# benjiebob/SMALify

Hardware: AMD Instinct MI355X
Metric: fitter iterations/sec (higher is better)
Workload: dtype f32

## Files before the change

### smalify_amd/csrc/kernels_raster.inc

```

#ifdef SMALFIT_DEV_PROBES
#define SMALFIT_PROBE(flags, bit) (((flags) & (bit)) != 0)
#else
#define SMALFIT_PROBE(flags, bit) false
#endif

#ifdef SMALFIT_WORK_STATS
__device__ unsigned long long g_work[32];
__device__ float g_probe_seed_scale;
#define SMALFIT_WORK(...) __VA_ARGS__
__device__ __forceinline__ void work_add(int slot, unsigned long long v) {
  unsigned lo = (unsigned)v, hi = (unsigned)(v >> 32);
#pragma unroll
  for (int o = 32; o > 0; o >>= 1) {
    const unsigned long long w = ((unsigned long long)__shfl_xor(hi, o, 64) << 32) | __shfl_xor(lo, o, 64);
    const unsigned long long s = (((unsigned long long)hi << 32) | lo) + w;
    lo = (unsigned)s; hi = (unsigned)(s >> 32);
  }
  if ((threadIdx.x & 63) == 0) atomicAdd(&g_work[slot], ((unsigned long long)hi << 32) | lo);
}
__device__ __forceinline__ int wave_max_i(int v) {
#pragma unroll
  for (int o = 32; o > 0; o >>= 1) v = max(v, __shfl_xor(v, o, 64));
  return v;
}
#else
#define SMALFIT_WORK(...)
#endif

constexpr int kListCap = 128;
constexpr int kListLds = 128;
static_assert(kListLds <= kListCap && kListLds % 8 == 0, "lists are copied out in 8-byte pieces");
constexpr int kMaskRounds = 64;
constexpr unsigned char kMaskList = 254;
constexpr unsigned char kNoList = 255;
constexpr float kBoxSlack = 1.0f / 64.0f;
constexpr int kTicketBase = 64, kTicketStride = 16;
constexpr int kQCountInts = kTicketBase + 8 * kSelGroups * kTicketStride;
constexpr int kAccWin = 36;
constexpr int kCountShift = 50;
constexpr float kLogFix = 16777216.0f;
constexpr int kBandCap = 64;
constexpr int kBandFill = 24;
constexpr int kBandFillWide = 40, kBandFillNarrow = 12;
constexpr int kBandStage = 64;
constexpr float kBandHalf = 4.0f;

struct SilTarget {
  const float* f;
  const unsigned char* b;
  __host__ __device__ explicit operator bool() const { return f != nullptr || b != nullptr; }
  __device__ __forceinline__ float operator[](size_t i) const { return b ? (float)b[i] / 255.0f : f[i]; }
};

__device__ __forceinline__ void xcd_block_of(int b , int blocks_per_frame, int& n, int& bx) {
  const int xcd = b & 7, slot = b >> 3;
  n = (slot / blocks_per_frame) * 8 + xcd;
  bx = slot - (slot / blocks_per_frame) * blocks_per_frame;
}
__device__ __forceinline__ void xcd_block(int blocks_per_frame, int& n, int& bx) { xcd_block_of((int)blockIdx.x, blocks_per_frame, n, bx); }

__device__ __forceinline__ unsigned orderable(float f) {
  const unsigned u = __float_as_uint(f);
  return (u & 0x80000000u) ? ~u : (u | 0x80000000u);
}
__device__ __forceinline__ float from_orderable(unsigned k) {
  return __uint_as_float((k & 0x80000000u) ? (k & 0x7fffffffu) : ~k);
}
__device__ __forceinline__ float wave_prod(float v) {
#pragma unroll
  for (int o = 32; o > 0; o >>= 1) v *= __shfl_xor(v, o, 64);
  return v;
}
__device__ __forceinline__ bool box_contains(int2 b, int x, int y) {
  return (b.x & 0xffff) <= x && x <= (b.x >> 16) && (b.y & 0xffff) <= y && y <= (b.y >> 16);
}
__device__ __forceinline__ unsigned long long pack_candidate(float d) {
  const float x2 = d * (1.4426950408889634f / kSigma);
  const float t = __builtin_amdgcn_exp2f(-fabsf(x2));
  const float f = fminf(__builtin_amdgcn_logf(1.0f + t) - fminf(x2, 0.0f), 255.99998f);
  return (1ull << kCountShift) | (unsigned long long)(unsigned)fmaf(f, kLogFix, 0.5f);
}

struct PixelSeed { float sil, adiff, gx; };
__device__ __forceinline__ PixelSeed pixel_no_target(float alpha) { return {1.0f - alpha, 0.f, 0.f}; }
__device__ __forceinline__ PixelSeed pixel_seed(float alpha, float ts, float wn) {
  PixelSeed p = pixel_no_target(alpha);
  const float diff = p.sil - ts;
  p.adiff = fabsf(diff);
  const float sgn = (diff > 0.f) ? 1.0f : ((diff < 0.f) ? -1.0f : 0.0f);
  p.gx = -wn * sgn * alpha * (1.0f / kSigma);
  return p;
}

__device__ __forceinline__ float prob_fast(float d) {
  return __builtin_amdgcn_rcpf(1.0f + __builtin_amdgcn_exp2f(d * (1.4426950408889634f / kSigma)));
}

constexpr int kRecVecs = 4;
__device__ __forceinline__ void store_face_rec(float4* __restrict__ o, const FaceRec& r) {
  o[0] = make_float4(r.ax, r.ay, r.e1x, r.e1y);
  o[1] = make_float4(r.e2x, r.e2y, r.e3x, r.e3y);
  o[2] = make_float4(r.il1, r.il2, r.il3, r.area);
  o[3] = make_float4(r.inv_den, r.pz0, r.gzx, r.gzy);
}
__device__ __forceinline__ void unpack_face_rec(const float4 a, const float4 b, const float4 c, const float4 d, FaceRec& r) {
  r.ax = a.x; r.ay = a.y; r.e1x = a.z; r.e1y = a.w;
  r.e2x = b.x; r.e2y = b.y; r.e3x = b.z; r.e3y = b.w;
  r.il1 = c.x; r.il2 = c.y; r.il3 = c.z; r.area = c.w;
  r.t01 = (c.x == 0.0f) ? 1.0f : 0.0f; r.t02 = (c.y == 0.0f) ? 1.0f : 0.0f; r.t03 = (c.z == 0.0f) ? 1.0f : 0.0f;
  r.inv_den = d.x; r.pz0 = d.y; r.gzx = d.z; r.gzy = d.w; r.pad = 0.0f;
}
__device__ __forceinline__ void load_face_rec(const float4* __restrict__ fr, FaceRec& r) {
  const float4 a = fr[0], b = fr[1], c = fr[2], d = fr[3];
  unpack_face_rec(a, b, c, d, r);
}

__global__ void __launch_bounds__(256)
face_bbox_kernel(ModelDev m, int M, int S, const float* __restrict__ proj, int2* __restrict__ fbox,
                 float4* __restrict__ frec , int4* __restrict__ brect ,
                 float* __restrict__ zc , int* __restrict__ frect ,
                 int* __restrict__ qcount ,
                 const float* __restrict__ jverts, float* __restrict__ joints_out ) {
  const int nfr = box_frame_blocks(M);
  const int Vp = m.Vp;
  if ((int)blockIdx.x < nfr) {
    const int n = (int)blockIdx.x;
    if (n >= M) return;
    if (n == 0) {
      if (threadIdx.x < 3) qcount[threadIdx.x] = 0;
      for (int i = threadIdx.x; i < 8 * kSelGroups; i += 256) qcount[kTicketBase + i * kTicketStride] = 0;
    }
    const float* px = proj + (size_t)n * 3 * Vp;
    if (threadIdx.x < 64) {
      const float zsum = wave_sum(px[2 * Vp + (int)(((long long)threadIdx.x * m.V) >> 6)]);
      if (threadIdx.x == 0) zc[n] = zsum * (1.0f / 64.0f);
    }
    __shared__ float rr[4][4];
    float xlo = 3.0e38f, xhi = -3.0e38f, ylo = 3.0e38f, yhi = -3.0e38f;
#pragma unroll 8
    for (int v = threadIdx.x; v < m.V; v += 256) {
      const float x = px[v], y = px[Vp + v];
      xlo = fminf(xlo, x); xhi = fmaxf(xhi, x); ylo = fminf(ylo, y); yhi = fmaxf(yhi, y);
    }
#pragma unroll
    for (int o = 32; o > 0; o >>= 1) {
      xlo = fminf(xlo, __shfl_xor(xlo, o, 64)); xhi = fmaxf(xhi, __shfl_xor(xhi, o, 64));
      ylo = fminf(ylo, __shfl_xor(ylo, o, 64)); yhi = fmaxf(yhi, __shfl_xor(yhi, o, 64));
    }
    if ((threadIdx.x & 63) == 0) { float* q = rr[threadIdx.x >> 6]; q[0] = xlo; q[1] = xhi; q[2] = ylo; q[3] = yhi; }
    __syncthreads();
    if (threadIdx.x == 0) {
      for (int w = 1; w < 4; ++w) { xlo = fminf(xlo, rr[w][0]); xhi = fmaxf(xhi, rr[w][1]); ylo = fminf(ylo, rr[w][2]); yhi = fmaxf(yhi, rr[w][3]); }
      xlo -= kBlurSqrt; xhi += kBlurSqrt; ylo -= kBlurSqrt; yhi += kBlurSqrt;
      const float fs = (float)S;
      const float c0 = fmaxf(floorf(((1.0f - xhi) * fs - 1.0f) * 0.5f), 0.f), c1 = fminf(ceilf(((1.0f - xlo) * fs - 1.0f) * 0.5f), fs - 1.f);
      const float r0 = fmaxf(floorf(((1.0f - yhi) * fs - 1.0f) * 0.5f), 0.f), r1 = fminf(ceilf(((1.0f - ylo) * fs - 1.0f) * 0.5f), fs - 1.f);
      int4 o = make_int4(0, 0, 0, 0);
      if (c0 <= c1 && r0 <= r1) o = make_int4(S - (int)c0, (int)c1 + 1, S - (int)r0, (int)r1 + 1);
      *reinterpret_cast<int4*>(frect + n * 4) = o;
    }
    return;
  }
  const int nbb = box_face_blocks(m.F, M);
  if ((int)blockIdx.x >= nfr + nbb) {
    __shared__ float jred[16];
    const int k = (int)blockIdx.x - nfr - nbb;
    joints_block(m, jverts, joints_out, k % kJointBlocks, k / kJointBlocks, jred);
    return;
  }
  int n, bxi;
  xcd_block_of((int)blockIdx.x - nfr, box_blocks_per_frame(m.F), n, bxi);
  if (n >= M) return;
  __shared__ __attribute__((aligned(16))) float4 recs[256][kRecVecs];
  const int f = bxi * 256 + threadIdx.x;
  const float* px = proj + (size_t)n * 3 * Vp;
  int2 box = make_int2(1, 1);
  if (f < m.F) {
    const int i0 = m.faces[f * 3], i1 = m.faces[f * 3 + 1], i2 = m.faces[f * 3 + 2];
    const float ax = px[i0], ay = px[Vp + i0], az = px[2 * Vp + i0];
    const float bx = px[i1], by = px[Vp + i1], bz = px[2 * Vp + i1];
    const float cx = px[i2], cy = px[Vp + i2], cz = px[2 * Vp + i2];
    FaceRec r;
    const bool ok = make_face_rec(ax, ay, az, bx, by, bz, cx, cy, cz, r);
    if (ok) {
      const float xlo = fminf(ax, fminf(bx, cx)) - kBlurSqrt, xhi = fmaxf(ax, fmaxf(bx, cx)) + kBlurSqrt;
      const float ylo = fminf(ay, fminf(by, cy)) - kBlurSqrt, yhi = fmaxf(ay, fmaxf(by, cy)) + kBlurSqrt;
      const float fs = (float)S;
      float c0 = ceilf(((1.0f - xhi) * fs - 1.0f) * 0.5f - kBoxSlack);
      float c1 = floorf(((1.0f - xlo) * fs - 1.0f) * 0.5f + kBoxSlack);
      float r0 = ceilf(((1.0f - yhi) * fs - 1.0f) * 0.5f - kBoxSlack);
      float r1 = floorf(((1.0f - ylo) * fs - 1.0f) * 0.5f + kBoxSlack);
      c0 = fminf(fmaxf(c0, 0.f), fs - 1.f); c1 = fminf(fmaxf(c1, -1.f), fs - 1.f);
      r0 = fminf(fmaxf(r0, 0.f), fs - 1.f); r1 = fminf(fmaxf(r1, -1.f), fs - 1.f);
      const bool finite = (xlo == xlo) && (xhi == xhi) && (ylo == ylo) && (yhi == yhi);
      const bool onscreen = finite && (xhi >= -1.0f) && (xlo <= 1.0f) && (yhi >= -1.0f) && (ylo <= 1.0f) &&
                            (c1 >= c0) && (r1 >= r0);
      if (onscreen) box = make_int2((int)c0 | ((int)c1 << 16), (int)r0 | ((int)r1 << 16));
    }
    fbox[(size_t)n * m.F + f] = box;
    store_face_rec(&recs[threadIdx.x][0], r);
  }
  __syncthreads();
  {
    const int nrec = min(256, m.F - bxi * 256);
    float4* dst = frec + ((size_t)n * m.F + (size_t)bxi * 256) * kRecVecs;
#pragma unroll
    for (int q = 0; q < kRecVecs; ++q) {
      const int idx = q * 256 + (int)threadIdx.x;
      if (idx < nrec * kRecVecs) dst[idx] = recs[idx >> 2][idx & 3];
    }
  }
  const bool live = (box.x & 0xffff) <= (box.x >> 16);
  int x0 = live ? (box.x & 0xffff) : 0x7fff, x1 = live ? (box.x >> 16) : -1;
  int y0 = live ? (box.y & 0xffff) : 0x7fff, y1 = live ? (box.y >> 16) : -1;
#pragma unroll
  for (int o = kRectFaces / 2; o > 0; o >>= 1) {
    x0 = min(x0, __shfl_xor(x0, o, kRectFaces)); x1 = max(x1, __shfl_xor(x1, o, kRectFaces));
    y0 = min(y0, __shfl_xor(y0, o, kRectFaces)); y1 = max(y1, __shfl_xor(y1, o, kRectFaces));
  }
  if ((threadIdx.x & (kRectFaces - 1)) == 0 && f < m.F)
    brect[(size_t)n * rect_count(m.F) + f / kRectFaces] = make_int4(x0, x1, y0, y1);
}

__global__ void __launch_bounds__(256, 1)
raster_sweep_kernel(int F, int M, int S, const float4* __restrict__ frec, const int2* __restrict__ fbox, const int4* __restrict__ brect, const float* __restrict__ zc, const float2* __restrict__ zband,
                    unsigned long long* __restrict__ gacc , unsigned* __restrict__ bcnt ,
                    float2* __restrict__ blist , unsigned char* __restrict__ plist ,
                    unsigned char* __restrict__ pcount ) {
  static_assert(kSweepFaces % kRectFaces == 0, "a sweep block is a whole number of union boxes");
  __shared__ __attribute__((aligned(16))) float4 raw[kSweepFaces][kRecVecs];
  __shared__ int2 boxes[kSweepFaces];
  __shared__ unsigned long long acc[kAccWin * kAccWin];
  __shared__ float2 st_e[4][kBandStage];
  __shared__ int st_p[4][kBandStage];
  __shared__ int st_n[4];
  __shared__ __attribute__((aligned(8))) unsigned char lsts[kSweepFaces][kListLds];
  __shared__ int lcn[kSweepFaces];
  static_assert(sizeof(raw) + sizeof(boxes) + sizeof(acc) + sizeof(st_e) + sizeof(st_p) + sizeof(st_n) + sizeof(lsts) + sizeof(lcn)
                <= 160 * 1024 / 8, "eight sweep workgroups per CU (160 KB of LDS)");
  const int t = threadIdx.x;
  int n, bxi;
  xcd_block(sweep_blocks_per_frame(F), n, bxi);
  if (n >= M) return;
  const int f0 = bxi * kSweepFaces;
  SMALFIT_WORK(const unsigned long long ws_t0 = __builtin_amdgcn_s_memtime();)
  int rect[4] = {0x7fff, -1, 0x7fff, -1};
  {
    const int nrect = rect_count(F);
    const int4* br = brect + (size_t)n * nrect + (size_t)bxi * (kSweepFaces / kRectFaces);
#pragma unroll
    for (int u = 0; u < kSweepFaces / kRectFaces; ++u) {
      if (bxi * (kSweepFaces / kRectFaces) + u < nrect) {
        const int4 b = br[u];
        rect[0] = min(rect[0], b.x); rect[1] = max(rect[1], b.y); rect[2] = min(rect[2], b.z); rect[3] = max(rect[3], b.w);
      }
    }
  }
  float4 q4 = make_float4(0.f, 0.f, 0.f, 0.f);
  int2 bq = make_int2(1, 1);
  const bool ld_rec = t < kSweepFaces * kRecVecs && f0 + (t >> 2) < F;
  const bool ld_box = t >= 128 && t < 128 + kSweepFaces && f0 + (t - 128) < F;
  static_assert(kSweepFaces * kRecVecs <= 128 && kRecVecs == 4, "record quarters by threads 0..127, boxes by 128..159");
  if (ld_rec) q4 = frec[((size_t)n * F + f0) * kRecVecs + t];
  if (ld_box) bq = fbox[(size_t)n * F + f0 + (t - 128)];
  if (t < 4) st_n[t] = 0;
  if (t < kSweepFaces) lcn[t] = 0;
  {
    const int zrows = min(kAccWin, max(rect[3] - rect[2] + 1, 0));
    for (int i = t; i < zrows * kAccWin; i += 256) acc[i] = 0ull;
  }
  SMALFIT_WORK(const unsigned long long ws_t1 = __builtin_amdgcn_s_memtime();)
  if (t < kSweepFaces * kRecVecs) raw[t >> 2][t & 3] = q4;
  if (t >= 128 && t < 128 + kSweepFaces) {
    boxes[t - 128] = bq;
    if (ld_box && (bq.x & 0xffff) > (bq.x >> 16)) pcount[(size_t)n * F + f0 + (t - 128)] = 0;
  }
  __syncthreads();
  SMALFIT_WORK(const unsigned long long ws_t2 = __builtin_amdgcn_s_memtime();)
  if (rect[1] < rect[0]) return;
  const int rw = rect[1] - rect[0] + 1, rh = rect[3] - rect[2] + 1;
  const int wx0 = rect[0] + max(0, (rw - kAccWin) >> 1), wy0 = rect[2] + max(0, (rh - kAccWin) >> 1);
  const float wx0f = (float)wx0, wy0f = (float)wy0;
  const bool clip = rw > kAccWin || rh > kAccWin;
  constexpr float hwin = 0.5f * (float)(kAccWin - 1);
  const size_t fbase = (size_t)n * S * S;
  unsigned long long* ga = gacc + fbase;
  const float2* zbp = zband + fbase;
  const int sub = t & 15, grp = t >> 4;
  const float inv_s = 1.0f / (float)S;
  const int wv = t >> 6, lane = t & 63;
  float zcn = zc[n];
  asm volatile("" : "+v"(zcn));
  auto flush_band = [&]() {
    const int cnt = min(__builtin_amdgcn_readfirstlane(st_n[wv]), kBandStage);
    for (int i = lane; i < cnt; i += 64) {
      const size_t pi = fbase + (size_t)st_p[wv][i];
      const unsigned slot = atomicAdd(&bcnt[pi], 1u);
      if (slot < (unsigned)kBandCap) blist[pi * kBandCap + slot] = st_e[wv][i];
    }
    __builtin_amdgcn_wave_barrier();
    if (lane == 0) st_n[wv] = 0;
    __builtin_amdgcn_fence(__ATOMIC_ACQ_REL, "wavefront");
    __builtin_amdgcn_wave_barrier();
  };
  SMALFIT_WORK(int ws_vis = 0; int ws_depth = 0; int ws_eval = 0; int ws_near = 0; int ws_trips = 0; int ws_rounds = 0; int ws_clipped = 0;)
#pragma unroll 1
  for (int step = 0; step < kSweepFaces / 16; ++step) {
    SMALFIT_WORK(ws_rounds += wave_max_i(ws_trips); ws_trips = 0;)
    if (__builtin_amdgcn_readfirstlane(st_n[wv]) >= kBandStage / 2) flush_band();
    const int k = step * 16 + grp;
    const int2 box = boxes[k];
    const int c0 = box.x & 0xffff, c1 = box.x >> 16, r0 = box.y & 0xffff, r1 = box.y >> 16;
    if (c0 > c1) continue;
    FaceRec rk;
    unpack_face_rec(raw[k][0], raw[k][1], raw[k][2], raw[k][3], rk);
    const int bw = c1 - c0 + 1, npx = bw * (r1 - r0 + 1);
    const bool listed = npx <= 256;
    unsigned long long lmask = 0ull, lbit = 1ull;
    const float bwf = (float)bw, ibw = __builtin_amdgcn_rcpf(bwf), hbw = 0.5f * ibw, npxf = (float)npx;
    const float r0f = (float)r0, c0f = (float)c0;
    const float ndc_a = -2.0f * inv_s, ndc_b = 1.0f - inv_s;
    const float s8 = 8.0f * (float)S;
    auto bounds_of = [&](float q) {
      const float ry = floorf(fmaf(q, ibw, hbw));
      const float rw = r0f + ry, cl = c0f + fmaf(-ry, bwf, q);
      return *reinterpret_cast<const float2*>(reinterpret_cast<const char*>(zbp) + (unsigned)fmaf(rw, s8, 8.0f * cl));
    };
    float2 zb_next = make_float2(0.f, 0.f);
    if ((float)sub < npxf) zb_next = bounds_of((float)sub);
    for (float qf = (float)sub; qf < npxf; qf += 16.0f, lbit <<= 1) {
      const float ryf = floorf(fmaf(qf, ibw, hbw));
      const float rowf = r0f + ryf, colf = c0f + fmaf(-ryf, bwf, qf);
      const unsigned boff = (unsigned)fmaf(rowf, s8, 8.0f * colf);
      const float2 zb = zb_next;
      if (qf + 16.0f < npxf) zb_next = bounds_of(qf + 16.0f);
      const float ppx = fmaf(colf, ndc_a, ndc_b), ppy = fmaf(rowf, ndc_a, ndc_b);
      const float rz = face_pixel_depth(rk, ppx, ppy) - zcn;
      SMALFIT_WORK(++ws_vis; ++ws_trips;)
      if (!(rz <= zb.y)) continue;
      SMALFIT_WORK(++ws_depth;)
      PixEval e;
      if (!face_pixel_candidate(rk, ppx, ppy, e.d)) continue;
      SMALFIT_WORK(++ws_eval;)
      lmask |= lbit;
      if (listed) {
        const int pos = atomicAdd(&lcn[k], 1);
        if (pos < kListLds) lsts[k][pos] = (unsigned char)(int)qf;
      }
      if (rz <= zb.x) {
        SMALFIT_WORK(++ws_near;)
        const float lxf = colf - wx0f, lyf = rowf - wy0f;
        if (!clip || (fabsf(lxf - hwin) <= hwin && fabsf(lyf - hwin) <= hwin))
          atomicAdd(reinterpret_cast<unsigned long long*>(reinterpret_cast<char*>(acc) + (unsigned)fmaf(lyf, 8.0f * (float)kAccWin, 8.0f * lxf)), pack_candidate(e.d));
        else { atomicAdd(reinterpret_cast<unsigned long long*>(reinterpret_cast<char*>(ga) + boff), pack_candidate(e.d)); SMALFIT_WORK(++ws_clipped;) }
      } else {
        const int sl = atomicAdd(&st_n[wv], 1);
        if (sl < kBandStage) {
          st_p[wv][sl] = (int)(boff >> 3);
          st_e[wv][sl] = make_float2(rz, e.d);
        } else {
          const size_t pi = fbase + (size_t)(boff >> 3);
          const unsigned slot = atomicAdd(&bcnt[pi], 1u);
          if (slot < (unsigned)kBandCap) blist[pi * kBandCap + slot] = make_float2(rz, e.d);
        }
      }
    }
    {
      int tt = threadIdx.x;
      asm volatile("" : "+v"(tt));
      const int sub2 = tt & 15, k2 = step * 16 + (tt >> 4);
      __builtin_amdgcn_fence(__ATOMIC_ACQ_REL, "wavefront");
      const int cnt = lcn[k2];
      const int2 bx = boxes[k2];
      const int npx2 = ((bx.x >> 16) - (bx.x & 0xffff) + 1) * ((bx.y >> 16) - (bx.y & 0xffff) + 1);
      int n2, bx2;
      xcd_block(sweep_blocks_per_frame(F), n2, bx2);
      const size_t fi = (size_t)n2 * F + bx2 * kSweepFaces + k2;
      const bool has_list = npx2 <= 256 && cnt <= kListLds;
      unsigned char flag;
      if (__ballot(!has_list) == 0ull) {
        flag = (unsigned char)cnt;
        if (sub2 * 8 < cnt) reinterpret_cast<uint2*>(plist + fi * kListCap)[sub2] = reinterpret_cast<const uint2*>(&lsts[k2][0])[sub2];
      } else if (npx2 <= 16 * kMaskRounds) {
        flag = kMaskList;
        reinterpret_cast<unsigned long long*>(plist + fi * kListCap)[sub2] = lmask;
      } else {
        flag = kNoList;
      }
      if (sub2 == 0) pcount[fi] = flag;
    }
  }
  SMALFIT_WORK(const unsigned long long ws_t3 = __builtin_amdgcn_s_memtime();)
  static_assert(kBandStage <= 64, "one staged band entry per lane in the final flush");
  const int fcnt = min(__builtin_amdgcn_readfirstlane(st_n[wv]), kBandStage);
  size_t fpi = 0;
  unsigned fslot = (unsigned)kBandCap;
  float2 fe = make_float2(0.f, 0.f);
  if (lane < fcnt) {
    fpi = fbase + (size_t)st_p[wv][lane];
    fe = st_e[wv][lane];
    fslot = atomicAdd(&bcnt[fpi], 1u);
  }
  __syncthreads();
  SMALFIT_WORK(const unsigned long long ws_t4 = __builtin_amdgcn_s_memtime();)
  SMALFIT_WORK(ws_rounds += wave_max_i(ws_trips); int ws_flush = 0;)
  const int ww = min(kAccWin, rect[1] - wx0 + 1), wh = min(kAccWin, rect[3] - wy0 + 1);
  for (int i = t; i < wh * kAccWin; i += 256) {
    const int lyw = i / kAccWin, lxw = i % kAccWin;
    if (lxw >= ww) continue;
    const unsigned long long v = acc[lyw * kAccWin + lxw];
    if (v) { atomicAdd(&ga[(wy0 + lyw) * S + wx0 + lxw], v); SMALFIT_WORK(++ws_flush;) }
  }
  if (fslot < (unsigned)kBandCap) blist[fpi * kBandCap + fslot] = fe;
  SMALFIT_WORK(work_add(0, ws_vis); work_add(1, ws_depth); work_add(2, ws_eval); work_add(3, ws_near); work_add(7, ws_clipped); work_add(31, (lane == 0 && clip) ? 1 : 0);
               work_add(4, lane == 0 ? ws_rounds : 0); work_add(5, ws_flush); work_add(6, lane == 0 ? 1 : 0);)
}

constexpr float kLossFix = 1099511627776.0f;
__device__ __forceinline__ long long wave_sum_i64(long long v) {
#pragma unroll
  for (int o = 32; o > 0; o >>= 1) {
    const int lo = __shfl_xor((int)(v & 0xffffffffll), o, 64), hi = __shfl_xor((int)(v >> 32), o, 64);
    v += ((long long)hi << 32) | (unsigned int)lo;
  }
  return v;
}

struct FrameLoss { long long acc; int n; };
__device__ __forceinline__ void frame_loss_flush(unsigned long long* floss, FrameLoss& f) {
// ... 856 lines not shown
```

### smalify_amd/csrc/smalfit_launch.inc

```
#include <algorithm>
#include <cstdio>
#include <cstring>
#include <string>
#include <vector>

#include "../../include/smalfit.h"
#include "smalfit_plan.h"
#include "smal_model_pack.h"

namespace smalfit {

static thread_local std::string g_err;
static_assert(kHeadPriorFrames == kPriorFrames, "smalfit_plan.h counts the prior blocks of lbs_head_images_kernel");
#ifdef SMALFIT_DEV_PROBES
static int g_dbg = 0;
#else
static constexpr int g_dbg = 0;
#endif

static int fail(const std::string& msg) {
  g_err = msg;
  return 1;
}
static int refused(const char* who, const char* why) { return why ? fail(std::string(who) + ": " + why) : 0; }
// ... 410 lines not shown
  PriorFrames pf;
  std::memset(&pf, 0, sizeof(pf));
  if (x.prior == HeadPrior::PerFrame) {
    pf.on = 1; pf.loss = e->loss_betas_pf; pf.gb = e->gb_prior_pf; pf.gb_stride = kPriorSlotB; pf.gls = e->gls_prior_pf; pf.gls_stride = kPriorSlotLs;
  }
  const int nhead = head_blocks(M, m.Vp, betas_stride != 0, x.prior);
  switch (x.head) {
    case HeadKernel::Step: lbs_head_step_kernel<<<nhead, 256, 0, st>>>(m, h, *x.pending); break;
    case HeadKernel::Images: lbs_head_images_kernel<<<nhead, 256, 0, st>>>(m, h, pf); break;
    case HeadKernel::Plain: lbs_head_kernel<<<nhead, 256, 0, st>>>(m, h); break;
  }
  LAUNCH_OK("lbs_head_kernel");
  const int vs_stride = betas_stride ? 3 * m.Vp : 0;
  const SkinForm form = skin_form(M, m.Vp);
  const Grid2 sg = skin_grid(form, M, m.Vp);
  switch (form) {
    case SkinForm::Wide:
      skin_mfma_kernel<<<dim3(sg.x, sg.y), 256, 0, st>>>(m, M, e->Mp, e->v_shaped, vs_stride, e->pfT, e->Am, trans, e->vposed, e->verts, e->proj);
      break;
    case SkinForm::Split:
      skin_mfma_split_kernel<<<dim3(sg.x, sg.y), kSkinThreads, 0, st>>>(m, M, e->Mp, e->v_shaped, vs_stride, e->pfT, e->Am, trans, e->vposed,
                                                                     e->verts, e->proj);
      break;
    case SkinForm::Plain:
      skin_kernel<8><<<dim3(sg.x, sg.y), 256, 0, st>>>(m, M, e->Mp, e->v_shaped, vs_stride, e->pfT, e->Am, trans, e->vposed, e->verts, e->proj);
      break;
  }
  LAUNCH_OK("skin_kernel");
  if (joints_out) {
    joints_kernel<<<dim3(kJointBlocks, M), 128, 0, st>>>(m, e->verts, joints_out);
    LAUNCH_OK("joints_kernel");
  }
  return 0;
}

template <typename... Args>
static void launch_raster_band(hipStream_t st, bool frame_loss, Args... args) {
  if (frame_loss) raster_band_kernel<true><<<kBandBlocks, 256, 0, st>>>(args...);
  else raster_band_kernel<false><<<kBandBlocks, 256, 0, st>>>(args...);
}
template <typename... Args>
static void launch_raster_select(hipStream_t st, bool frame_loss, Args... args) {
  if (frame_loss) raster_select_kernel<true><<<kSelectBlocks, 64 * kSelWaves, 0, st>>>(args...);
  else raster_select_kernel<false><<<kSelectBlocks, 64 * kSelWaves, 0, st>>>(args...);
}

static int run_raster_forward(smalfit_engine* e, hipStream_t st, int M, WinMap win, float w_sil,
                              SilTarget tsil, float* sil_out, float* blk_loss,
                              float* joints_out = nullptr, const LossArgs* la = nullptr, bool queue_loss = false,
                              unsigned long long* floss = nullptr) {
  float2* gz = e->gz;
  const ModelDev& m = e->model->dev;
  {
    Section sec(e, st, SMALFIT_SEC_RASTER_BBOX);
    face_bbox_kernel<<<box_grid(m.F, M, joints_out != nullptr), 256, 0, st>>>(m, M, e->S, e->proj, e->fbox, e->frec, e->brect, e->zc, e->frect,
                                                                           e->qcount, e->verts, joints_out);
    LAUNCH_OK("face_bbox_kernel");
  }
  {
    Section sec(e, st, SMALFIT_SEC_RASTER_SWEEP);
    raster_sweep_kernel<<<sweep_grid(m.F, M), 256, 0, st>>>(m.F, M, e->S, e->frec, e->fbox, e->brect, e->zc, e->zband, e->gacc, e->bcnt, e->blist, e->plist, e->pcount);
    LAUNCH_OK("raster_sweep_kernel");
  }
  {
    Section sec(e, st, SMALFIT_SEC_RASTER_RESOLVE);
    LossArgs no_loss;
    std::memset(&no_loss, 0, sizeof(no_loss));
    const int loss_frames = la ? M : 0;
    raster_resolve_kernel<<<resolve_grid(e->nrb, M, loss_frames), 256, 0, st>>>(e->S, M, win, w_sil, e->gacc, e->bcnt, e->frect, e->zband, tsil, sil_out, gz,
                                                                             blk_loss, e->qcount, e->queue, e->bqueue, g_dbg ? e->status : nullptr,
                                                                             la ? *la : no_loss, loss_frames);
    LAUNCH_OK("raster_resolve_kernel");
    launch_raster_band(st, floss != nullptr, e->S, M, win, w_sil, e->gacc, e->bcnt, e->blist, tsil, sil_out, gz, e->zband,
                       e->qcount, e->queue, e->bqueue, queue_loss ? e->qloss + kSelectBlocks : nullptr, floss);
    LAUNCH_OK("raster_band_kernel");
  }
  Section sec(e, st, SMALFIT_SEC_RASTER_SELECT);
  launch_raster_select(st, floss != nullptr, m.F, e->S, M, win, w_sil, e->frec, e->zc, e->brect, e->fbox, e->qcount, e->queue,
                       tsil, sil_out, gz, e->zband, e->pcount, queue_loss ? e->qloss : nullptr, g_dbg, floss);
  LAUNCH_OK("raster_select_kernel");
  return 0;
}

static int run_lbs_backward(smalfit_engine* e, hipStream_t st, int M, int nb, int betas_shared,
                            const float* dface, const float* dJ41, const float* dext, bool need_pose,
                            bool need_beta, bool need_ls, const float* dth_direct, int j_stride, float* dRs_out = nullptr) {
  const ModelDev& m = e->model->dev;
  vertex_bwd_kernel<<<vertex_bwd_grid(m.Vp, M), 256, 0, st>>>(m, M, e->proj, dface, dJ41, dext, e->Am, e->dvert, e->dvp, e->dtr_part);
  LAUNCH_OK("vertex_bwd_kernel");
  const int nPB = need_pose ? mid_pb_ids(M) : 0;
  const DbetaGrid db = dbeta_grid(need_beta, m.Vp, betas_shared != 0, M);
  lbs_bwd_mid_kernel<<<mid_grid(M, nPB), 256, 0, st>>>(m, M, nPB, e->dvert, e->vposed, e->dvp, e->dA, e->dpf_part);
  LAUNCH_OK("lbs_bwd_mid_kernel");
  chain_bwd_kernel<<<chain_grid(M, db), 256, 0, st>>>(m, M, e->theta, e->Rm, e->Gm, e->scm, e->Jrest, j_stride, e->dA,
                                                    need_pose ? e->dpf_part : nullptr, e->CS, dth_direct, e->dtheta,
                                                    need_ls ? e->dls : nullptr, e->dJrest, need_beta ? e->dbetaJ : nullptr, dRs_out,
                                                    nb, betas_shared, db.bx, db.by, db.bz, e->dvp, e->dbeta_part);
  LAUNCH_OK("chain_bwd_kernel");
  return 0;
}

static int launch_frame_betas_assembly(smalfit_engine* e, hipStream_t st, int M, int nb, float* g_betas) {
  const ModelDev& m = e->model->dev;
  AssembleArgs g;
  std::memset(&g, 0, sizeof(g));
  g.M = M; g.nb = nb; g.NBall = m.NBall; g.nblk_beta = e->nblk_beta; g.betas_shared = 0;
  g.dbeta_part = e->dbeta_part; g.dJrest = e->dJrest; g.JS = m.JS; g.dbetaJ = e->dbetaJ; g.ngrp_beta = 1; g.g_betas = g_betas;
  g.win = WinMap{1, 0, M};
  assemble_kernel<false><<<frame_betas_grid(M), 256, 0, st>>>(g, AssembleExt{});
  LAUNCH_OK("assemble_kernel");
  return 0;
}

}
// ... 675 lines not shown
```

### smalify_amd/csrc/smalfit_plan.h

```cpp
#pragma once
#include <algorithm>
#include <cmath>
#include <cstring>

#include "../../include/smalfit.h"

namespace smalfit {

constexpr int kBetaGroups = 8;
constexpr int kMaxImageSize = 1024;
constexpr int kHeadPriorFrames = 16;
constexpr int kMeshQueries = 64;
constexpr int kMeshThreads = 256;

inline int padded_verts(int V) { return (V + 255) / 256 * 256; }
inline int nblk_beta(int Vp) { return (3 * Vp + 255) / 256; }
inline int beta_groups(bool betas_shared) { return betas_shared ? kBetaGroups : 1; }

struct DbetaGrid {
  int bx, by, bz;
  int blocks() const { return bx * by * bz; }
};
inline DbetaGrid dbeta_grid(bool need_beta, int Vp, bool betas_shared, int M) {
  return {need_beta ? nblk_beta(Vp) : 0, betas_shared ? 1 : M, beta_groups(betas_shared)};
}
inline size_t dbeta_rows(int max_frames) { return (size_t)max_frames + kBetaGroups; }

enum class SkinForm { Plain = 0, Split = 1, Wide = 2 };
inline SkinForm skin_form(int M, int Vp) {
  if (M <= 4) return SkinForm::Plain;
  return (Vp / 64) * ((M + 15) / 16) >= 256 ? SkinForm::Wide : SkinForm::Split;
}

enum class HeadPrior { None = 0, Shared = 1, PerFrame = 2 };
inline int head_shape_blocks(int M, int Vp, bool shape_per_frame) { return Vp / 256 * (shape_per_frame ? M : 1); }
inline int head_prior_blocks(int M, HeadPrior prior) {
  return prior == HeadPrior::None ? 0 : (prior == HeadPrior::Shared ? 1 : (M + kHeadPriorFrames - 1) / kHeadPriorFrames);
}
inline int head_blocks(int M, int Vp, bool shape_per_frame, HeadPrior prior) {
  return M + head_shape_blocks(M, Vp, shape_per_frame) + head_prior_blocks(M, prior);
}

constexpr int xcd_frames(int M) { return ((M + 7) / 8) * 8; }
constexpr int xcd_grid(int blocks_per_frame, int M) { return blocks_per_frame * ((M + 7) / 8) * 8; }
constexpr int elem_blocks(long long elements) { return (int)((elements + 255) / 256); }
constexpr int vertex_blocks(int Vp) { return Vp / 256; }
constexpr int rigid_blocks(int count) { return (count + 63) / 64; }
struct Grid2 { int x, y; };
constexpr int color_face_blocks(int F) { return (F + 15) / 16; }
constexpr int kSilCountPixels = 16;
constexpr Grid2 cover_grid(int F, int M) { return Grid2{color_face_blocks(F), M}; }
constexpr int sil_count_slabs(int S) { return ((S * S + kSilCountPixels - 1) / kSilCountPixels + 255) / 256; }
constexpr Grid2 sil_counts_grid(int S, int M) { return Grid2{sil_count_slabs(S), M}; }
constexpr int pck_grid(int M) { return M; }

constexpr int kSkinGroups = 2;
constexpr int kSkinVerts = 16 * kSkinGroups;
constexpr int kSkinThreads = 256 * kSkinGroups;
constexpr Grid2 skin_grid(SkinForm form, int M, int Vp) {
  return form == SkinForm::Wide ? Grid2{Vp / 64, (M + 15) / 16} : form == SkinForm::Split ? Grid2{Vp / kSkinVerts, (M + 15) / 16} : Grid2{Vp / 64, (M + 7) / 8};
}
constexpr int kJointBlocks = 41;

constexpr int box_frame_blocks(int M) { return xcd_frames(M); }
constexpr int box_blocks_per_frame(int F) { return (F + 255) / 256; }
constexpr int box_face_blocks(int F, int M) { return xcd_grid(box_blocks_per_frame(F), M); }
constexpr int box_joint_blocks(int M, bool joints) { return joints ? kJointBlocks * M : 0; }
constexpr int box_grid(int F, int M, bool joints) { return box_frame_blocks(M) + box_face_blocks(F, M) + box_joint_blocks(M, joints); }

constexpr int kRectFaces = 8;
constexpr int kSweepFaces = 32;
constexpr int rect_count(int F) { return (F + kRectFaces - 1) / kRectFaces; }
constexpr int sweep_blocks_per_frame(int F) { return (F + kSweepFaces - 1) / kSweepFaces; }
constexpr int sweep_grid(int F, int M) { return xcd_grid(sweep_blocks_per_frame(F), M); }

constexpr int kResSub = 2;
constexpr int kResEdge = 16 * kResSub;
constexpr int resolve_tiles_x(int S) { return (S + kResEdge - 1) / kResEdge; }
constexpr int resolve_tiles(int S) { return resolve_tiles_x(S) * resolve_tiles_x(S); }
constexpr int resolve_loss_blocks(int loss_frames) { return loss_frames > 0 ? ((loss_frames + 7) / 8) * 8 : 0; }
constexpr int resolve_grid(int tiles, int M, int loss_frames) { return xcd_grid(tiles, M) + resolve_loss_blocks(loss_frames); }

constexpr int kBandBlocks = 1536;
constexpr int kSelWaves = 2;
constexpr int kSelGroups = 16;
constexpr int kSelectBlocks = 1792;
static_assert(kSelectBlocks % (8 * kSelGroups) == 0, "every ticket group of every XCD needs the same number of selection workgroups (a group without one would leave its pixels undone)");
constexpr int kQueueLossBlocks = kSelectBlocks + kBandBlocks;
constexpr int kFrameLossStride = 32;

constexpr int kBwdLanes = 16;
constexpr int kBwdFaces = 4;
constexpr int raster_bwd_blocks_per_frame(int F) { return (F + kBwdFaces - 1) / kBwdFaces; }
constexpr int raster_bwd_grid(int F, int M) { return xcd_grid(raster_bwd_blocks_per_frame(F), M); }
inline float raster_bwd_inv_s(int S) { return 1.0f / (float)S; }
constexpr int kMaxModelFaces = 1 << 25;

constexpr int vertex_bwd_grid(int Vp, int M) { return xcd_grid(vertex_blocks(Vp), M); }

constexpr int PBM_SPLITS = 24, PBM_TILES = 4;
static_assert(PBM_SPLITS % 8 == 0, "the blocks of a column split are placed on one XCD (ids in chunks of 8 splits)");
constexpr int mid_pb_ids(int M) { return 10 * PBM_SPLITS * (((M + 15) / 16 + PBM_TILES - 1) / PBM_TILES); }
constexpr int mid_da_ids(int M) { return xcd_grid(35, M); }
constexpr int mid_grid(int M, int nPB) { return (nPB ? mid_pb_ids(M) : 0) + mid_da_ids(M); }

inline int chain_grid(int M, const DbetaGrid& db) { return M + db.blocks(); }

constexpr int kAsmElem = 4, kAsmLoss = 16;
constexpr int kAsmRows = 4;
constexpr int asm_shape_sets(int betas_shared, int M) { return betas_shared ? 1 : M; }
constexpr int assemble_grid(int shape_sets) { return shape_sets + 1 + kAsmElem + kAsmLoss; }
constexpr int window_rows_grid(int W) { return W; }
constexpr int frame_loss_rows_grid() { return kAsmRows; }

inline bool parents_ordered(const int* parents, int num_joints) {
  for (int i = 1; i < num_joints; ++i)
    if (!(parents[i] >= 0 && parents[i] < i)) return false;
  return true;
}

constexpr int kTreeMaxPass = 16, kTreeMaxChildren = 4;
struct TreeLevels {
  unsigned char nlev;
  unsigned char lvl_off[36];
  unsigned char lvl_joint[35];
  unsigned char child_off[36];
  unsigned char child_idx[35];
// ... 833 lines not shown
```

Baseline: 2988.

## Fuse face bbox/record setup into raster sweep kernel, removing separate launch

Removes the face_bbox_kernel launch and folds its work into raster_sweep_kernel. Each sweep block now builds its own 32 face records and boxes in LDS directly from projected vertices, instead of writing them to global memory and reading them back. The block also computes the reference depth itself and writes the records out for later stages. Frame-region and joint blocks become extra roles in the same grid. This saves one kernel launch and a global round trip, but the reference depth is now recomputed in every sweep block and the face setup sits on the sweep's critical path.

```diff
diff --git a/smalify_amd/csrc/kernels_raster.inc b/smalify_amd/csrc/kernels_raster.inc
--- a/smalify_amd/csrc/kernels_raster.inc
+++ b/smalify_amd/csrc/kernels_raster.inc
@@ -54,9 +54,9 @@
 };
 
 __device__ __forceinline__ void xcd_block_of(int b , int blocks_per_frame, int& n, int& bx) {
-  const int xcd = b & 7, slot = b >> 3;
-  n = (slot / blocks_per_frame) * 8 + xcd;
-  bx = slot - (slot / blocks_per_frame) * blocks_per_frame;
+  const XcdBlock x = xcd_block_at(b, blocks_per_frame);
+  n = x.n;
+  bx = x.bx;
 }
 __device__ __forceinline__ void xcd_block(int blocks_per_frame, int& n, int& bx) { xcd_block_of((int)blockIdx.x, blocks_per_frame, n, bx); }
 
@@ -116,115 +116,71 @@
   unpack_face_rec(a, b, c, d, r);
 }
 
-__global__ void __launch_bounds__(256)
-face_bbox_kernel(ModelDev m, int M, int S, const float* __restrict__ proj, int2* __restrict__ fbox,
-                 float4* __restrict__ frec , int4* __restrict__ brect ,
-                 float* __restrict__ zc , int* __restrict__ frect ,
-                 int* __restrict__ qcount ,
-                 const float* __restrict__ jverts, float* __restrict__ joints_out ) {
-  const int nfr = box_frame_blocks(M);
+
+__device__ __forceinline__ float frame_ref_depth(const float* __restrict__ pz, int V, int lane) {
+  return wave_sum(pz[(int)(((long long)lane * V) >> 6)]) * (1.0f / 64.0f);
+}
+
+__device__ __forceinline__ int2 face_pixel_box(bool ok, float ax, float ay, float bx, float by, float cx, float cy, int S) {
+  int2 box = make_int2(1, 1);
+  if (ok) {
+    const float xlo = fminf(ax, fminf(bx, cx)) - kBlurSqrt, xhi = fmaxf(ax, fmaxf(bx, cx)) + kBlurSqrt;
+    const float ylo = fminf(ay, fminf(by, cy)) - kBlurSqrt, yhi = fmaxf(ay, fmaxf(by, cy)) + kBlurSqrt;
+    const float fs = (float)S;
+    float c0 = ceilf(((1.0f - xhi) * fs - 1.0f) * 0.5f - kBoxSlack);
+    float c1 = floorf(((1.0f - xlo) * fs - 1.0f) * 0.5f + kBoxSlack);
+    float r0 = ceilf(((1.0f - yhi) * fs - 1.0f) * 0.5f - kBoxSlack);
+    float r1 = floorf(((1.0f - ylo) * fs - 1.0f) * 0.5f + kBoxSlack);
+    c0 = fminf(fmaxf(c0, 0.f), fs - 1.f); c1 = fminf(fmaxf(c1, -1.f), fs - 1.f);
+    r0 = fminf(fmaxf(r0, 0.f), fs - 1.f); r1 = fminf(fmaxf(r1, -1.f), fs - 1.f);
+    const bool finite = (xlo == xlo) && (xhi == xhi) && (ylo == ylo) && (yhi == yhi);
+    const bool onscreen = finite && (xhi >= -1.0f) && (xlo <= 1.0f) && (yhi >= -1.0f) && (ylo <= 1.0f) &&
+                          (c1 >= c0) && (r1 >= r0);
+    if (onscreen) box = make_int2((int)c0 | ((int)c1 << 16), (int)r0 | ((int)r1 << 16));
+  }
+  return box;
+}
+
+__device__ __forceinline__ void frame_region_block(const ModelDev& m, int S, const float* __restrict__ proj, int* __restrict__ frect,
+                                                   int* __restrict__ qcount, int n, float (*rr)[4] ) {
   const int Vp = m.Vp;
-  if ((int)blockIdx.x < nfr) {
-    const int n = (int)blockIdx.x;
-    if (n >= M) return;
-    if (n == 0) {
-      if (threadIdx.x < 3) qcount[threadIdx.x] = 0;
-      for (int i = threadIdx.x; i < 8 * kSelGroups; i += 256) qcount[kTicketBase + i * kTicketStride] = 0;
-    }
-    const float* px = proj + (size_t)n * 3 * Vp;
-    if (threadIdx.x < 64) {
-      const float zsum = wave_sum(px[2 * Vp + (int)(((long long)threadIdx.x * m.V) >> 6)]);
-      if (threadIdx.x == 0) zc[n] = zsum * (1.0f / 64.0f);
-    }
-    __shared__ float rr[4][4];
-    float xlo = 3.0e38f, xhi = -3.0e38f, ylo = 3.0e38f, yhi = -3.0e38f;
+  if (n == 0) {
+    if (threadIdx.x < 3) qcount[threadIdx.x] = 0;
+    for (int i = threadIdx.x; i < 8 * kSelGroups; i += 256) qcount[kTicketBase + i * kTicketStride] = 0;
+  }
+  const float* px = proj + (size_t)n * 3 * Vp;
+  float xlo = 3.0e38f, xhi = -3.0e38f, ylo = 3.0e38f, yhi = -3.0e38f;
 #pragma unroll 8
-    for (int v = threadIdx.x; v < m.V; v += 256) {
-      const float x = px[v], y = px[Vp + v];
-      xlo = fminf(xlo, x); xhi = fmaxf(xhi, x); ylo = fminf(ylo, y); yhi = fmaxf(yhi, y);
-    }
-#pragma unroll
-    for (int o = 32; o > 0; o >>= 1) {
-      xlo = fminf(xlo, __shfl_xor(xlo, o, 64)); xhi = fmaxf(xhi, __shfl_xor(xhi, o, 64));
-      ylo = fminf(ylo, __shfl_xor(ylo, o, 64)); yhi = fmaxf(yhi, __shfl_xor(yhi, o, 64));
-    }
-    if ((threadIdx.x & 63) == 0) { float* q = rr[threadIdx.x >> 6]; q[0] = xlo; q[1] = xhi; q[2] = ylo; q[3] = yhi; }
-    __syncthreads();
-    if (threadIdx.x == 0) {
-      for (int w = 1; w < 4; ++w) { xlo = fminf(xlo, rr[w][0]); xhi = fmaxf(xhi, rr[w][1]); ylo = fminf(ylo, rr[w][2]); yhi = fmaxf(yhi, rr[w][3]); }
-      xlo -= kBlurSqrt; xhi += kBlurSqrt; ylo -= kBlurSqrt; yhi += kBlurSqrt;
-      const float fs = (float)S;
-      const float c0 = fmaxf(floorf(((1.0f - xhi) * fs - 1.0f) * 0.5f), 0.f), c1 = fminf(ceilf(((1.0f - xlo) * fs - 1.0f) * 0.5f), fs - 1.f);
-      const float r0 = fmaxf(floorf(((1.0f - yhi) * fs - 1.0f) * 0.5f), 0.f), r1 = fminf(ceilf(((1.0f - ylo) * fs - 1.0f) * 0.5f), fs - 1.f);
-      int4 o = make_int4(0, 0, 0, 0);
-      if (c0 <= c1 && r0 <= r1) o = make_int4(S - (int)c0, (int)c1 + 1, S - (int)r0, (int)r1 + 1);
-      *reinterpret_cast<int4*>(frect + n * 4) = o;
-    }
-    return;
-  }
-  const int nbb = box_face_blocks(m.F, M);
-  if ((int)blockIdx.x >= nfr + nbb) {
-    __shared__ float jred[16];
-    const int k = (int)blockIdx.x - nfr - nbb;
-    joints_block(m, jverts, joints_out, k % kJointBlocks, k / kJointBlocks, jred);
-    return;
-  }
-  int n, bxi;
-  xcd_block_of((int)blockIdx.x - nfr, box_blocks_per_frame(m.F), n, bxi);
-  if (n >= M) return;
-  __shared__ __attribute__((aligned(16))) float4 recs[256][kRecVecs];
-  const int f = bxi * 256 + threadIdx.x;
-  const float* px = proj + (size_t)n * 3 * Vp;
-  int2 box = make_int2(1, 1);
-  if (f < m.F) {
-    const int i0 = m.faces[f * 3], i1 = m.faces[f * 3 + 1], i2 = m.faces[f * 3 + 2];
-    const float ax = px[i0], ay = px[Vp + i0], az = px[2 * Vp + i0];
-    const float bx = px[i1], by = px[Vp + i1], bz = px[2 * Vp + i1];
-    const float cx = px[i2], cy = px[Vp + i2], cz = px[2 * Vp + i2];
-    FaceRec r;
-    const bool ok = make_face_rec(ax, ay, az, bx, by, bz, cx, cy, cz, r);
-    if (ok) {
-      const float xlo = fminf(ax, fminf(bx, cx)) - kBlurSqrt, xhi = fmaxf(ax, fmaxf(bx, cx)) + kBlurSqrt;
-      const float ylo = fminf(ay, fminf(by, cy)) - kBlurSqrt, yhi = fmaxf(ay, fmaxf(by, cy)) + kBlurSqrt;
-      const float fs = (float)S;
-      float c0 = ceilf(((1.0f - xhi) * fs - 1.0f) * 0.5f - kBoxSlack);
-      float c1 = floorf(((1.0f - xlo) * fs - 1.0f) * 0.5f + kBoxSlack);
-      float r0 = ceilf(((1.0f - yhi) * fs - 1.0f) * 0.5f - kBoxSlack);
-      float r1 = floorf(((1.0f - ylo) * fs - 1.0f) * 0.5f + kBoxSlack);
-      c0 = fminf(fmaxf(c0, 0.f), fs - 1.f); c1 = fminf(fmaxf(c1, -1.f), fs - 1.f);
-      r0 = fminf(fmaxf(r0, 0.f), fs - 1.f); r1 = fminf(fmaxf(r1, -1.f), fs - 1.f);
-      const bool finite = (xlo == xlo) && (xhi == xhi) && (ylo == ylo) && (yhi == yhi);
-      const bool onscreen = finite && (xhi >= -1.0f) && (xlo <= 1.0f) && (yhi >= -1.0f) && (ylo <= 1.0f) &&
-                            (c1 >= c0) && (r1 >= r0);
-      if (onscreen) box = make_int2((int)c0 | ((int)c1 << 16), (int)r0 | ((int)r1 << 16));
-    }
-    fbox[(size_t)n * m.F + f] = box;
-    store_face_rec(&recs[threadIdx.x][0], r);
-  }
+  for (int v = threadIdx.x; v < m.V; v += 256) {
+    const float x = px[v], y = px[Vp + v];
+    xlo = fminf(xlo, x); xhi = fmaxf(xhi, x); ylo = fminf(ylo, y); yhi = fmaxf(yhi, y);
+  }
+#pragma unroll
+  for (int o = 32; o > 0; o >>= 1) {
+    xlo = fminf(xlo, __shfl_xor(xlo, o, 64)); xhi = fmaxf(xhi, __shfl_xor(xhi, o, 64));
+    ylo = fminf(ylo, __shfl_xor(ylo, o, 64)); yhi = fmaxf(yhi, __shfl_xor(yhi, o, 64));
+  }
+  if ((threadIdx.x & 63) == 0) { float* q = rr[threadIdx.x >> 6]; q[0] = xlo; q[1] = xhi; q[2] = ylo; q[3] = yhi; }
   __syncthreads();
-  {
-    const int nrec = min(256, m.F - bxi * 256);
-    float4* dst = frec + ((size_t)n * m.F + (size_t)bxi * 256) * kRecVecs;
-#pragma unroll
-    for (int q = 0; q < kRecVecs; ++q) {
-      const int idx = q * 256 + (int)threadIdx.x;
-      if (idx < nrec * kRecVecs) dst[idx] = recs[idx >> 2][idx & 3];
-    }
-  }
-  const bool live = (box.x & 0xffff) <= (box.x >> 16);
-  int x0 = live ? (box.x & 0xffff) : 0x7fff, x1 = live ? (box.x >> 16) : -1;
-  int y0 = live ? (box.y & 0xffff) : 0x7fff, y1 = live ? (box.y >> 16) : -1;
-#pragma unroll
-  for (int o = kRectFaces / 2; o > 0; o >>= 1) {
-    x0 = min(x0, __shfl_xor(x0, o, kRectFaces)); x1 = max(x1, __shfl_xor(x1, o, kRectFaces));
-    y0 = min(y0, __shfl_xor(y0, o, kRectFaces)); y1 = max(y1, __shfl_xor(y1, o, kRectFaces));
-  }
-  if ((threadIdx.x & (kRectFaces - 1)) == 0 && f < m.F)
-    brect[(size_t)n * rect_count(m.F) + f / kRectFaces] = make_int4(x0, x1, y0, y1);
+  if (threadIdx.x == 0) {
+    for (int w = 1; w < 4; ++w) { xlo = fminf(xlo, rr[w][0]); xhi = fmaxf(xhi, rr[w][1]); ylo = fminf(ylo, rr[w][2]); yhi = fmaxf(yhi, rr[w][3]); }
+    xlo -= kBlurSqrt; xhi += kBlurSqrt; ylo -= kBlurSqrt; yhi += kBlurSqrt;
+    const float fs = (float)S;
+    const float c0 = fmaxf(floorf(((1.0f - xhi) * fs - 1.0f) * 0.5f), 0.f), c1 = fminf(ceilf(((1.0f - xlo) * fs - 1.0f) * 0.5f), fs - 1.f);
+    const float r0 = fmaxf(floorf(((1.0f - yhi) * fs - 1.0f) * 0.5f), 0.f), r1 = fminf(ceilf(((1.0f - ylo) * fs - 1.0f) * 0.5f), fs - 1.f);
+    int4 o = make_int4(0, 0, 0, 0);
+    if (c0 <= c1 && r0 <= r1) o = make_int4(S - (int)c0, (int)c1 + 1, S - (int)r0, (int)r1 + 1);
+    *reinterpret_cast<int4*>(frect + n * 4) = o;
+  }
 }
 
 __global__ void __launch_bounds__(256, 1)
-raster_sweep_kernel(int F, int M, int S, const float4* __restrict__ frec, const int2* __restrict__ fbox, const int4* __restrict__ brect, const float* __restrict__ zc, const float2* __restrict__ zband,
+raster_sweep_kernel(ModelDev m, int M, int S, const float* __restrict__ proj, float4* __restrict__ frec ,
+                    int2* __restrict__ fbox , int4* __restrict__ brect , float* __restrict__ zc ,
+                    int* __restrict__ frect ,
+                    int* __restrict__ qcount ,
+                    const float* __restrict__ jverts, float* __restrict__ joints_out ,
+                    const float2* __restrict__ zband,
                     unsigned long long* __restrict__ gacc , unsigned* __restrict__ bcnt ,
                     float2* __restrict__ blist , unsigned char* __restrict__ plist ,
                     unsigned char* __restrict__ pcount ) {
@@ -237,47 +193,86 @@
   __shared__ int st_n[4];
   __shared__ __attribute__((aligned(8))) unsigned char lsts[kSweepFaces][kListLds];
   __shared__ int lcn[kSweepFaces];
-  static_assert(sizeof(raw) + sizeof(boxes) + sizeof(acc) + sizeof(st_e) + sizeof(st_p) + sizeof(st_n) + sizeof(lsts) + sizeof(lcn)
-                <= 160 * 1024 / 8, "eight sweep workgroups per CU (160 KB of LDS)");
+  __shared__ int4 brect_s;
+  __shared__ float zc_s;
+  static_assert(sizeof(raw) + sizeof(boxes) + sizeof(acc) + sizeof(st_e) + sizeof(st_p) + sizeof(st_n) + sizeof(lsts) + sizeof(lcn) +
+                sizeof(brect_s) + 16  <= 160 * 1024 / 8, "eight sweep workgroups per CU (160 KB of LDS)");
   const int t = threadIdx.x;
-  int n, bxi;
-  xcd_block(sweep_blocks_per_frame(F), n, bxi);
+  const int F = m.F;
+  const SweepBlock role = sweep_block_at((int)blockIdx.x, F, M);
+  if (role.role != SweepRole::Faces) {
+    if (role.role == SweepRole::Joint) joints_block(m, jverts, joints_out, role.bx, role.n, reinterpret_cast<float*>(acc));
+    else if (role.n < M) frame_region_block(m, S, proj, frect, qcount, role.n, reinterpret_cast<float (*)[4]>(acc));
+    return;
+  }
+  const int n = role.n, bxi = role.bx;
   if (n >= M) return;
   const int f0 = bxi * kSweepFaces;
   SMALFIT_WORK(const unsigned long long ws_t0 = __builtin_amdgcn_s_memtime();)
-  int rect[4] = {0x7fff, -1, 0x7fff, -1};
-  {
-    const int nrect = rect_count(F);
-    const int4* br = brect + (size_t)n * nrect + (size_t)bxi * (kSweepFaces / kRectFaces);
-#pragma unroll
-    for (int u = 0; u < kSweepFaces / kRectFaces; ++u) {
-      if (bxi * (kSweepFaces / kRectFaces) + u < nrect) {
-        const int4 b = br[u];
-        rect[0] = min(rect[0], b.x); rect[1] = max(rect[1], b.y); rect[2] = min(rect[2], b.z); rect[3] = max(rect[3], b.w);
-      }
-    }
-  }
-  float4 q4 = make_float4(0.f, 0.f, 0.f, 0.f);
-  int2 bq = make_int2(1, 1);
-  const bool ld_rec = t < kSweepFaces * kRecVecs && f0 + (t >> 2) < F;
-  const bool ld_box = t >= 128 && t < 128 + kSweepFaces && f0 + (t - 128) < F;
-  static_assert(kSweepFaces * kRecVecs <= 128 && kRecVecs == 4, "record quarters by threads 0..127, boxes by 128..159");
-  if (ld_rec) q4 = frec[((size_t)n * F + f0) * kRecVecs + t];
-  if (ld_box) bq = fbox[(size_t)n * F + f0 + (t - 128)];
-  if (t < 4) st_n[t] = 0;
-  if (t < kSweepFaces) lcn[t] = 0;
-  {
-    const int zrows = min(kAccWin, max(rect[3] - rect[2] + 1, 0));
-    for (int i = t; i < zrows * kAccWin; i += 256) acc[i] = 0ull;
+  static_assert(kSweepFaces * kRecVecs <= 128 && kRecVecs == 4 && kSweepFaces <= 32, "faces by threads 0..31; record quarters leave by threads 0..127, boxes by 128..159");
+  const float* px = proj + (size_t)n * 3 * m.Vp;
+  if ((__builtin_amdgcn_readfirstlane(t) >> 6) == 0) {
+    __builtin_amdgcn_s_setprio(3);
+    if (t < kSweepFaces) {
+      const int Vp = m.Vp;
+      const int f = f0 + t;
+      int2 box = make_int2(1, 1);
+      if (f < F) {
+        const int i0 = m.faces[f * 3], i1 = m.faces[f * 3 + 1], i2 = m.faces[f * 3 + 2];
+        const float ax = px[i0], ay = px[Vp + i0], az = px[2 * Vp + i0];
+        const float bx = px[i1], by = px[Vp + i1], bz = px[2 * Vp + i1];
+        const float cx = px[i2], cy = px[Vp + i2], cz = px[2 * Vp + i2];
+        FaceRec r;
+        const bool ok = make_face_rec(ax, ay, az, bx, by, bz, cx, cy, cz, r);
+        box = face_pixel_box(ok, ax, ay, bx, by, cx, cy, S);
+        store_face_rec(&raw[t][0], r);
+      }
+      boxes[t] = box;
+      lcn[t] = 0;
+      const bool live = (box.x & 0xffff) <= (box.x >> 16);
+      int x0 = live ? (box.x & 0xffff) : 0x7fff, x1 = live ? (box.x >> 16) : -1;
+      int y0 = live ? (box.y & 0xffff) : 0x7fff, y1 = live ? (box.y >> 16) : -1;
+#pragma unroll
+      for (int o = kRectFaces / 2; o > 0; o >>= 1) {
+        x0 = min(x0, __shfl_xor(x0, o, kRectFaces)); x1 = max(x1, __shfl_xor(x1, o, kRectFaces));
+        y0 = min(y0, __shfl_xor(y0, o, kRectFaces)); y1 = max(y1, __shfl_xor(y1, o, kRectFaces));
+      }
+      if ((t & (kRectFaces - 1)) == 0 && f < F)
+        brect[(size_t)n * rect_count(F) + f / kRectFaces] = make_int4(x0, x1, y0, y1);
+#pragma unroll
+      for (int o = kSweepFaces / 2; o >= kRectFaces; o >>= 1) {
+        x0 = min(x0, __shfl_xor(x0, o, kSweepFaces)); x1 = max(x1, __shfl_xor(x1, o, kSweepFaces));
+        y0 = min(y0, __shfl_xor(y0, o, kSweepFaces)); y1 = max(y1, __shfl_xor(y1, o, kSweepFaces));
+      }
+      if (t == 0) brect_s = make_int4(x0, x1, y0, y1);
+    }
+    __builtin_amdgcn_s_setprio(0);
+  } else {
+    float zcv = 0.f;
+    if (t < 128) zcv = frame_ref_depth(px + 2 * m.Vp, m.V, t - 64);
+    for (int i = t - 64; i < kAccWin * kAccWin; i += 192) acc[i] = 0ull;
+    if (t == 64) {
+      zc_s = zcv;
+      if (bxi == 0) zc[n] = zcv;
+    }
+    if (t >= 128 && t < 132) st_n[t - 128] = 0;
   }
   SMALFIT_WORK(const unsigned long long ws_t1 = __builtin_amdgcn_s_memtime();)
-  if (t < kSweepFaces * kRecVecs) raw[t >> 2][t & 3] = q4;
-  if (t >= 128 && t < 128 + kSweepFaces) {
-    boxes[t - 128] = bq;
-    if (ld_box && (bq.x & 0xffff) > (bq.x >> 16)) pcount[(size_t)n * F + f0 + (t - 128)] = 0;
-  }
   __syncthreads();
   SMALFIT_WORK(const unsigned long long ws_t2 = __builtin_amdgcn_s_memtime();)
+  int rect[4];
+  {
+    const int4 b = brect_s;
+    rect[0] = __builtin_amdgcn_readfirstlane(b.x); rect[1] = __builtin_amdgcn_readfirstlane(b.y);
+    rect[2] = __builtin_amdgcn_readfirstlane(b.z); rect[3] = __builtin_amdgcn_readfirstlane(b.w);
+  }
+  if (t < kSweepFaces * kRecVecs) {
+    if (f0 + (t >> 2) < F) frec[((size_t)n * F + f0) * kRecVecs + t] = raw[t >> 2][t & 3];
+  } else if (t < 128 + kSweepFaces && f0 + (t - 128) < F) {
+    const int2 bq = boxes[t - 128];
+    fbox[(size_t)n * F + f0 + (t - 128)] = bq;
+    if ((bq.x & 0xffff) > (bq.x >> 16)) pcount[(size_t)n * F + f0 + (t - 128)] = 0;
+  }
   if (rect[1] < rect[0]) return;
   const int rw = rect[1] - rect[0] + 1, rh = rect[3] - rect[2] + 1;
   const int wx0 = rect[0] + max(0, (rw - kAccWin) >> 1), wy0 = rect[2] + max(0, (rh - kAccWin) >> 1);
@@ -290,7 +285,7 @@
   const int sub = t & 15, grp = t >> 4;
   const float inv_s = 1.0f / (float)S;
   const int wv = t >> 6, lane = t & 63;
-  float zcn = zc[n];
+  float zcn = zc_s;
   asm volatile("" : "+v"(zcn));
   auto flush_band = [&]() {
     const int cnt = min(__builtin_amdgcn_readfirstlane(st_n[wv]), kBandStage);
@@ -375,7 +370,7 @@
       const int2 bx = boxes[k2];
       const int npx2 = ((bx.x >> 16) - (bx.x & 0xffff) + 1) * ((bx.y >> 16) - (bx.y & 0xffff) + 1);
       int n2, bx2;
-      xcd_block(sweep_blocks_per_frame(F), n2, bx2);
+      xcd_block_of((int)blockIdx.x - box_frame_blocks(M), sweep_blocks_per_frame(F), n2, bx2);
       const size_t fi = (size_t)n2 * F + bx2 * kSweepFaces + k2;
       const bool has_list = npx2 <= 256 && cnt <= kListLds;
       unsigned char flag;
diff --git a/smalify_amd/csrc/smalfit_launch.inc b/smalify_amd/csrc/smalfit_launch.inc
--- a/smalify_amd/csrc/smalfit_launch.inc
+++ b/smalify_amd/csrc/smalfit_launch.inc
@@ -486,14 +486,10 @@
   float2* gz = e->gz;
   const ModelDev& m = e->model->dev;
   {
-    Section sec(e, st, SMALFIT_SEC_RASTER_BBOX);
-    face_bbox_kernel<<<box_grid(m.F, M, joints_out != nullptr), 256, 0, st>>>(m, M, e->S, e->proj, e->fbox, e->frec, e->brect, e->zc, e->frect,
-                                                                           e->qcount, e->verts, joints_out);
-    LAUNCH_OK("face_bbox_kernel");
-  }
-  {
     Section sec(e, st, SMALFIT_SEC_RASTER_SWEEP);
-    raster_sweep_kernel<<<sweep_grid(m.F, M), 256, 0, st>>>(m.F, M, e->S, e->frec, e->fbox, e->brect, e->zc, e->zband, e->gacc, e->bcnt, e->blist, e->plist, e->pcount);
+    raster_sweep_kernel<<<sweep_launch_grid(m.F, M, joints_out != nullptr), 256, 0, st>>>(m, M, e->S, e->proj, e->frec, e->fbox, e->brect, e->zc, e->frect,
+                                                                                      e->qcount, e->verts, joints_out, e->zband, e->gacc, e->bcnt,
+                                                                                      e->blist, e->plist, e->pcount);
     LAUNCH_OK("raster_sweep_kernel");
   }
   {
diff --git a/smalify_amd/csrc/smalfit_plan.h b/smalify_amd/csrc/smalfit_plan.h
--- a/smalify_amd/csrc/smalfit_plan.h
+++ b/smalify_amd/csrc/smalfit_plan.h
@@ -68,11 +68,26 @@
 constexpr int box_joint_blocks(int M, bool joints) { return joints ? kJointBlocks * M : 0; }
 constexpr int box_grid(int F, int M, bool joints) { return box_frame_blocks(M) + box_face_blocks(F, M) + box_joint_blocks(M, joints); }
 
+struct XcdBlock { int n, bx; };
+constexpr XcdBlock xcd_block_at(int b, int blocks_per_frame) {
+  const int xcd = b & 7, slot = b >> 3;
+  return XcdBlock{(slot / blocks_per_frame) * 8 + xcd, slot - (slot / blocks_per_frame) * blocks_per_frame};
+}
+
 constexpr int kRectFaces = 8;
 constexpr int kSweepFaces = 32;
 constexpr int rect_count(int F) { return (F + kRectFaces - 1) / kRectFaces; }
 constexpr int sweep_blocks_per_frame(int F) { return (F + kSweepFaces - 1) / kSweepFaces; }
 constexpr int sweep_grid(int F, int M) { return xcd_grid(sweep_blocks_per_frame(F), M); }
+constexpr int sweep_launch_grid(int F, int M, bool joints) { return box_frame_blocks(M) + sweep_grid(F, M) + box_joint_blocks(M, joints); }
+enum class SweepRole { Frame = 0, Faces = 1, Joint = 2 };
+struct SweepBlock { SweepRole role; int n, bx; };
+constexpr SweepBlock sweep_block_at(int b, int F, int M) {
+  if (b < box_frame_blocks(M)) return SweepBlock{SweepRole::Frame, b, 0};
+  const int k = b - box_frame_blocks(M);
+  if (k >= sweep_grid(F, M)) return SweepBlock{SweepRole::Joint, (k - sweep_grid(F, M)) / kJointBlocks, (k - sweep_grid(F, M)) % kJointBlocks};
+  return SweepBlock{SweepRole::Faces, xcd_block_at(k, sweep_blocks_per_frame(F)).n, xcd_block_at(k, sweep_blocks_per_frame(F)).bx};
+}
 
 constexpr int kResSub = 2;
 constexpr int kResEdge = 16 * kResSub;
```

Result: faster. 3033, median of 6 (+1.5%).
